# jc-bao/gym-formation

Hardware: AMD Instinct MI355X
Metric: env-steps/sec (higher is better)
Workload: dtype f32

## Files before the change

gym-formation_amd/csrc/fg_obs_writers.hpp:

```cpp
#ifndef FG_OBS_WRITERS_HPP_
#define FG_OBS_WRITERS_HPP_

#include "fg_common.hpp"

namespace fg {

template <class V2> FG_DEV V2 lds_if(bool c, const V2* __restrict__ p, int idx_if_true) {
    V2 t = p[c ? idx_if_true : 0];
    t.x = c ? t.x : 0.0f; t.y = c ? t.y : 0.0f;
    return t;
}

constexpr bool FG_ROWS_MERGED = true;
template <int NC, int NW, int E, int PACE = 0>
FG_DEV void write_obs_rows(const real2* __restrict__ tables0, int env_stride, int w,
                           real2* __restrict__ out_env0, size_t env_units, int El, int parts,
                           int wg_part = 0, int wg_parts = 1, bool pace_on = true) {
    constexpr int N = NC;
    constexpr int WPE = (E >= NW) ? 1 : NW / E;
    constexpr int ESTEP = (E >= NW) ? NW : 1;
    static_assert((E >= NW) ? (E % NW == 0) : (NW % E == 0), "waves and envs must tile");
    const int lane = threadIdx.x & 63;
    const int row0 = (E >= NW) ? 0 : w % WPE;
    constexpr unsigned ROWU = 3u * N;
    for (int ee = (E >= NW) ? w : w / WPE; ee < El; ee += (E >= NW ? ESTEP : E)) {
        const real2* __restrict__ AA = tables0 + (size_t)ee * env_stride;
        real2* __restrict__ out = out_env0 + (size_t)ee * env_units;
        if constexpr (N <= 64) {
            constexpr int RW = 64 / N;
            const int rsub = lane / N, u = lane - rsub * N;
            const bool act = rsub < RW;
            const real2 zero = make_real2(0.f, 0.f);
            const real2 Pm = lds_if(act && u >= 1, AA, u - 1);
            const real2 Pu = lds_if(act && u >= 1, AA, u);
            const int xoff = (u == 0) ? 4 * N : 0;
            constexpr int CS = (2 * N + 63) / 64;
            constexpr int RS = (2 * N <= 64) ? 64 / (2 * N) : 1;
            const int ssub = (2 * N <= 64) ? lane / (2 * N) : 0;
            const int sidx = (2 * N <= 64) ? lane - ssub * 2 * N : lane;
            real2 sv[CS];
#pragma unroll
            for (int c = 0; c < CS; ++c)
                sv[c] = lds_if(ssub < RS && sidx + 64 * c < 2 * N, AA, N + sidx + 64 * c);
#pragma unroll 2
            for (int rb = row0; rb < N; rb += RW * WPE) {
                const int r = rb + rsub * WPE;
                if ((parts & 1) && act && r < N) {
                    const real2 x = AA[xoff + r];
                    const real2 c = (u - 1 >= r) ? Pu : Pm;
                    out[(unsigned)r * ROWU + (unsigned)u] = make_real2(c.x - x.x, c.y - x.y);
                }
#pragma unroll
                for (int k0 = 0; k0 < RW; k0 += RS) {
                    const int rs = rb + (k0 + ssub) * WPE;
                    if ((parts & 2) && ssub < RS && k0 + ssub < RW && rs < N) {
#pragma unroll
                        for (int c = 0; c < CS; ++c)
                            if (sidx + 64 * c < 2 * N) out[(unsigned)rs * ROWU + (unsigned)(N + sidx + 64 * c)] = sv[c];
                    }
                }
            }
        } else if constexpr (FG_ROWS_MERGED && ((3 * N + 63) / 64 < (N + 63) / 64 + (2 * N + 63) / 64)) {
            constexpr int CR = (3 * N + 63) / 64;
            constexpr int C_MIX = N / 64;
            real2 Pm[CR], Pu[CR];
#pragma unroll
            for (int c = 0; c < CR; ++c) {
                const int u = lane + 64 * c;
                if (c <= C_MIX) {
                    const bool dyn = u >= 1 && u < N, stat = u >= N && u < 3 * N;
                    Pm[c] = lds_if(dyn || stat, AA, stat ? u : u - 1);
                    Pu[c] = lds_if(dyn || stat, AA, u);
                } else {
                    Pm[c] = Pu[c] = lds_if(u < 3 * N, AA, u);
                }
            }
            const int nshare = WPE * wg_parts, share = wg_part * WPE + row0;
            const int PER = (N + nshare - 1) / nshare;
            const int r_end = min(N, (share + 1) * PER);
#pragma unroll 2
            for (int r = share * PER; r < r_end; ++r) {
                const real2 xp = AA[r];
                const real2 x0 = AA[(lane == 0 ? 4 * N : 0) + r];
                real2* __restrict__ orow = out + (unsigned)r * ROWU;
#pragma unroll
                for (int c = 0; c < CR; ++c) {
                    const int u = lane + 64 * c;
                    real2 val;
                    if (c < C_MIX || (c == C_MIX && (N % 64) == 0)) {
                        const real2 x = (c == 0) ? x0 : xp;
                        const real2 cc = (u - 1 >= r) ? Pu[c] : Pm[c];
                        val = make_real2(cc.x - x.x, cc.y - x.y);
                    } else if (c == C_MIX) {
                        const bool dyn = u < N;
                        const real2 x = (c == 0) ? x0 : xp;
                        const real2 cc = (u - 1 >= r) ? Pu[c] : Pm[c];
                        val = make_real2(cc.x - (dyn ? x.x : 0.0f), cc.y - (dyn ? x.y : 0.0f));
                    } else {
                        val = Pu[c];
                    }
                    if (u < 3 * N) orow[u] = val;
                }
                if (PACE > 0 && pace_on) __builtin_amdgcn_s_sleep(PACE);
            }
        } else {
            constexpr int CD = (N + 63) / 64, CS = (2 * N + 63) / 64;
            const real2 zero = make_real2(0.f, 0.f);
            real2 Pm[CD], Pu[CD], sv[CS];
#pragma unroll
            for (int c = 0; c < CD; ++c) {
                const int u = lane + 64 * c;
                Pm[c] = lds_if(u >= 1 && u < N, AA, u - 1);
                Pu[c] = lds_if(u >= 1 && u < N, AA, u);
            }
#pragma unroll
            for (int c = 0; c < CS; ++c) sv[c] = lds_if(lane + 64 * c < 2 * N, AA, N + lane + 64 * c);
            const int nshare = WPE * wg_parts, share = wg_part * WPE + row0;
            const int PER = (N + nshare - 1) / nshare;
            const int r_end = min(N, (share + 1) * PER);
#pragma unroll 2
            for (int r = share * PER; r < r_end; ++r) {
                const real2 xp = AA[r];
                const real2 x0 = AA[(lane == 0 ? 4 * N : 0) + r];
                real2* __restrict__ orow = out + (unsigned)r * ROWU;
#pragma unroll
                for (int c = 0; c < CD; ++c) {
                    const int u = lane + 64 * c;
                    const real2 x = (c == 0) ? x0 : xp;
                    const real2 cc = (u - 1 >= r) ? Pu[c] : Pm[c];
                    if ((parts & 1) && u < N) orow[u] = make_real2(cc.x - x.x, cc.y - x.y);
                }
#pragma unroll
                for (int c = 0; c < CS; ++c)
                    if ((parts & 2) && lane + 64 * c < 2 * N) orow[N + lane + 64 * c] = sv[c];
                if (PACE > 0 && pace_on) __builtin_amdgcn_s_sleep(PACE);
            }
        }
    }
}

template <int NC, int RT> constexpr int tile_units() { return (3 * NC * RT + 16 + 2 + 1) & ~1; }

template <int NC, int NW, int E, int RT, bool STREAM>
FG_DEV void write_obs_tiled(const float2* __restrict__ tables0, int env_stride, int w, float2* __restrict__ tiles,
                            float2* __restrict__ out_env0, size_t unit0, size_t env_units, int El) {
    constexpr int N = NC;
    constexpr int WPE = (E >= NW) ? 1 : NW / E;
    static_assert((E >= NW) ? (E % NW == 0) : (NW % E == 0), "waves and envs must tile");
    static_assert(N <= 32 && N % RT == 0, "tiled writer: N <= 32, RT divides N");
    constexpr unsigned ROWU = 3u * N, TU = ROWU * RT;
    constexpr int TILES_ENV = N / RT;
    constexpr int MY_TILES = (TILES_ENV + WPE - 1) / WPE;
    const int lane = threadIdx.x & 63;
    float2* tile0 = tiles + w * 2 * tile_units<NC, RT>();
    constexpr int RW = 64 / N;
    const int rsub = lane / N, u = lane - rsub * N;
    const bool act = rsub < RW;
    const int xoff = (u == 0) ? 4 * N : 0;
    constexpr int RS = 64 / (2 * N);
    const int ssub = lane / (2 * N), sidx = lane - ssub * 2 * N;
    const int e_first = (E >= NW) ? w : w / WPE, e_step = (E >= NW) ? NW : E;
    const int t_first = (E >= NW) ? 0 : w % WPE;
    const int n_env = (El > e_first) ? (El - e_first + e_step - 1) / e_step : 0;
    const int total = n_env * MY_TILES;

    constexpr unsigned ENVU = ROWU * N;
    const unsigned pad = (unsigned)(env_units - ENVU);
    static_assert(!STREAM || (E >= NW && NC >= 16), "streaming form: waves own whole envs, rows of >= 16 units");
    const bool own = STREAM && ((unit0 & 15) == 0) && (pad == 0 || (pad < 16 && (env_units & 15) == 0));
    auto head_units = [&](int ee) -> unsigned {
        return (own && pad == 0) ? (16u - (unsigned)(((size_t)ee * env_units) & 15)) & 15u : 0u;
    };
    auto extra_units = [&](int ee) -> unsigned {
        if (!own) return 0u;
        if (pad) return pad;
        return (ee + 1 < El) ? head_units(ee + 1) : 0u;
    };

    int cur_env = -1;
    const float2* __restrict__ AA = tables0;
    float2 Pm = make_float2(0.f, 0.f), Pu = Pm, sv = Pm;
    auto locate = [&](int t, int& ee, int& r0) {
        const int ie = t / MY_TILES, it = t - ie * MY_TILES;
        ee = e_first + ie * e_step;
        r0 = (t_first + it * WPE) * RT;
    };
    auto compose = [&](int t) {
        int ee, r0; locate(t, ee, r0);
        if (r0 >= N) return;
        if (ee != cur_env) {
            cur_env = ee;
            AA = tables0 + (size_t)ee * env_stride;
            Pm = lds_if(act && u >= 1, AA, u - 1);
            Pu = lds_if(act && u >= 1, AA, u);
            sv = lds_if(ssub < RS, AA, N + sidx);
        }
        const unsigned par = (unsigned)((unit0 + (size_t)ee * env_units + (size_t)r0 * ROWU) & 1);
        float2* img = tile0 + (t & 1) * tile_units<NC, RT>() + par;
#pragma unroll
        for (int rb = 0; rb < RT; rb += RW) {
            const int rl = rb + rsub;
            if (act && rl < RT) {
                const int r = r0 + rl;
                const float2 x = AA[xoff + r];
                const float2 c = (u - 1 >= r) ? Pu : Pm;
                img[(unsigned)rl * ROWU + (unsigned)u] = make_float2(c.x - x.x, c.y - x.y);
            }
        }
#pragma unroll
        for (int rb = 0; rb < RT; rb += RS) {
            const int rl = rb + ssub;
            if (ssub < RS && rl < RT) img[(unsigned)rl * ROWU + (unsigned)(N + sidx)] = sv;
        }
        if (STREAM && r0 + RT == N) {
            const unsigned x = extra_units(ee);
            if ((unsigned)lane < x) {
                float2 val = make_float2(0.f, 0.f);
                if (pad == 0) {
                    static_assert(ROWU >= 16, "the line remainder must stay inside row 0 of the next env");
                    const float2* __restrict__ A1 = tables0 + (size_t)(ee + 1) * env_stride;
                    const float2 a = A1[lane == 0 ? 3 * N : lane], b = A1[0];
                    const bool rel = lane >= 1 && lane < N;
                    val = make_float2(a.x - (rel ? b.x : 0.f), a.y - (rel ? b.y : 0.f));
                }
                img[TU + (unsigned)lane] = val;
            }
        }
    };
    auto stream = [&](int t) {
        int ee, r0; locate(t, ee, r0);
        if (r0 >= N) return;
        const unsigned par = (unsigned)((unit0 + (size_t)ee * env_units + (size_t)r0 * ROWU) & 1);
        const float2* img = tile0 + (t & 1) * tile_units<NC, RT>() + par;
        float2* __restrict__ out = out_env0 + (size_t)ee * env_units + (size_t)r0 * ROWU;
        if constexpr (!STREAM) {
            if (par && lane == 0) out[0] = img[0];
            constexpr unsigned NPMAX = TU >> 1;
            const unsigned npair = (TU - par) >> 1;
            const f32x4* src4 = reinterpret_cast<const f32x4*>(img + par);
            f32x4* __restrict__ dst4 = reinterpret_cast<f32x4*>(out + par);
#pragma unroll
            for (unsigned q0 = 0; q0 < NPMAX; q0 += 64) {
                const unsigned q = q0 + lane;
                if (q < npair) dst4[q] = src4[q];
            }
            if (((TU - par) & 1u) && lane == 63) out[TU - 1] = img[TU - 1];
        } else {
            const unsigned s = (r0 == 0) ? head_units(ee) : 0u;
            const unsigned end = TU + ((r0 + RT == N) ? extra_units(ee) : 0u);
            const unsigned p2 = (par + s) & 1u;
            if (p2 && lane == 0) out[s] = img[s];
            constexpr unsigned NPMAX = (TU + 16) >> 1;
            const unsigned npair = (end - s - p2) >> 1;
            const f32x4* src4 = reinterpret_cast<const f32x4*>(img + s + p2);
            f32x4* __restrict__ dst4 = reinterpret_cast<f32x4*>(out + s + p2);
            constexpr unsigned NFULL = ((TU - 16) >> 1) / 64;
#pragma unroll
            for (unsigned c = 0; c < NFULL; ++c) {
                const f32x4 v = src4[c * 64 + lane];
                asm volatile("s_waitcnt lgkmcnt(0)" ::: "memory");
                dst4[c * 64 + lane] = v;
                asm volatile("" ::: "memory");
                __builtin_amdgcn_s_sleep(1);
            }
#pragma unroll
            for (unsigned q0 = NFULL * 64; q0 < NPMAX; q0 += 64) {
                const unsigned q = q0 + lane;
                if (q < npair) dst4[q] = src4[q];
            }
            if (((end - s - p2) & 1u) && lane == 63) out[end - 1] = img[end - 1];
        }
    };
    if (total > 0) compose(0);
    for (int t = 0; t < total; ++t) {
        if (t + 1 < total) compose(t + 1);
        stream(t);
    }
}

constexpr int FG_WR_GATHER = 64;
template <int NC> constexpr int gather_passes() { return (3 * NC * NC / 2 + 2 + 63) / 64; }
template <int NC> constexpr int gather_lut_units() { return 2 * gather_passes<NC>() * 64 * 2; }

template <int NC>
FG_DEV void build_gather_lut(uint4* __restrict__ lut, int t, int nthreads) {
    constexpr int N = NC, ROWU = 3 * N, TU = ROWU * N, P = gather_passes<NC>() * 64;
    static_assert(N >= 2 && 5 * N < 65536, "gather writer: table offsets are 16-bit, the table's zeros are the 0 operand");
    auto operands = [&](int unit, unsigned& a, unsigned& b) {
        const int r = unit / ROWU, u = unit - r * ROWU;
        if (u == 0) { a = N; b = 4 * N + r; }
        else if (u < N) { a = (u - 1 >= r) ? u : u - 1; b = r; }
        else { a = u; b = N; }
    };
    for (int e = t; e < 2 * P; e += nthreads) {
        const int par = e / P, q = e - par * P;
        const int npair = (TU - par) >> 1;
        const bool tail = ((TU - par) & 1) != 0;
        int unit = -1, kind = 0;
        if (q < npair) { unit = 2 * q + par; kind = 2; }
        else if (par && q == npair) { unit = 0; kind = 1; }
        else if (tail && q == npair + par) { unit = TU - 1; kind = 1; }
        unsigned a0 = N, b0 = N, a1 = N, b1 = N;
        if (kind >= 1) operands(unit, a0, b0);
        if (kind == 2) operands(unit + 1, a1, b1);
        lut[e] = make_uint4(a0 | (b0 << 16), a1 | (b1 << 16), (unsigned)(unit < 0 ? 0 : unit) | ((unsigned)kind << 16), 0u);
    }
}

template <int NC> struct GatherEntries {
    uint32_t ab0[gather_passes<NC>()], ab1[gather_passes<NC>()], dst[gather_passes<NC>()];
    int phase = -1;
};

template <int NC, int NW, int E>
FG_DEV void write_obs_gather(const float2* __restrict__ tables0, int env_stride, int w, const uint4* __restrict__ lut,
                             float2* __restrict__ out_env0, size_t unit0, size_t env_units, int El, GatherEntries<NC>& cache) {
    constexpr int PASSES = gather_passes<NC>(), P = PASSES * 64;
    const int lane = threadIdx.x & 63;
    for (int ee = w; ee < El; ee += NW) {
        const float2* __restrict__ T = tables0 + (size_t)ee * env_stride;
        const size_t first = unit0 + (size_t)ee * env_units;
        float2* __restrict__ out = out_env0 + (size_t)ee * env_units;
        const int phase = (int)(first & 1);
        if (phase != cache.phase) {
            const uint4* __restrict__ L = lut + phase * P + lane;
#pragma unroll
            for (int c = 0; c < PASSES; ++c) {
                const uint4 t = L[c * 64];
                cache.ab0[c] = t.x; cache.ab1[c] = t.y; cache.dst[c] = t.z;
            }
            cache.phase = phase;
        }
        f32x4 val[PASSES];
#pragma unroll
        for (int c = 0; c < PASSES; ++c) {
            const float2 A0 = T[cache.ab0[c] & 0xffffu], B0 = T[cache.ab0[c] >> 16], A1 = T[cache.ab1[c] & 0xffffu], B1 = T[cache.ab1[c] >> 16];
            val[c] = (f32x4){A0.x - B0.x, A0.y - B0.y, A1.x - B1.x, A1.y - B1.y};
        }
#pragma unroll
        for (int c = 0; c < PASSES; ++c) {
            const unsigned kind = cache.dst[c] >> 16, dst = cache.dst[c] & 0xffffu;
            if (kind == 2) *reinterpret_cast<f32x4*>(out + dst) = val[c];
            else if (kind == 1) out[dst] = make_float2(val[c].x, val[c].y);
        }
    }
}

template <int NC, int NW, int E, int CHMAX = 4> struct SpanGather {
    static constexpr int ENVU = 3 * NC * NC, PIECES = E * ENVU / 2, INSTR = (PIECES + 63) / 64, MINE = (INSTR + NW - 1) / NW;
    static_assert((E * ENVU) % 2 == 0, "an even number of units per workgroup span");
    static FG_DEV void setup(uint2* __restrict__ lut, int w, int env_stride) {
        const int lane = threadIdx.x & 63;
        auto operands = [&](int unit) -> uint32_t {
            const int e = unit / ENVU, q = unit - e * ENVU;
            const int r = q / (3 * NC), u = q - r * (3 * NC);
            uint32_t a, b;
            if (u == 0) { a = NC; b = 4 * NC + r; }
            else if (u < NC) { a = (u - 1 >= r) ? u : u - 1; b = r; }
            else { a = u; b = NC; }
            const uint32_t base = (uint32_t)(e * env_stride);
            return (a + base) | ((b + base) << 16);
        };
        for (int t = 0; t < MINE; ++t) {
            const int piece = (w + NW * t) * 64 + lane;
            if (piece < PIECES) lut[piece] = make_uint2(operands(2 * piece), operands(2 * piece + 1));
        }
    }
    static FG_DEV void write(const uint2* __restrict__ lut, const float2* __restrict__ tables0, int w, float2* __restrict__ out) {
        const int lane = threadIdx.x & 63;
        f32x4* const out4 = reinterpret_cast<f32x4*>(out);
        constexpr int CH = MINE < CHMAX ? MINE : CHMAX;
#pragma unroll
        for (int t0 = 0; t0 < MINE; t0 += CH) {
            uint2 ent[CH];
#pragma unroll
            for (int c = 0; c < CH; ++c) {
                const int piece = (w + NW * (t0 + c)) * 64 + lane;
                ent[c] = lut[(t0 + c < MINE && piece < PIECES) ? piece : 0];
            }
            f32x4 val[CH];
#pragma unroll
            for (int c = 0; c < CH; ++c) {
                const float2 A0 = tables0[ent[c].x & 0xffffu], B0 = tables0[ent[c].x >> 16];
                const float2 A1 = tables0[ent[c].y & 0xffffu], B1 = tables0[ent[c].y >> 16];
                val[c] = (f32x4){A0.x - B0.x, A0.y - B0.y, A1.x - B1.x, A1.y - B1.y};
            }
#pragma unroll
            for (int c = 0; c < CH; ++c) {
                const int piece = (w + NW * (t0 + c)) * 64 + lane;
                if (t0 + c < MINE && piece < PIECES) out4[piece] = val[c];
            }
        }
    }
};

}

#endif
```

gym-formation_amd/csrc/fg_rollout_kernels.hpp:

```cpp
#ifndef FG_ROLLOUT_KERNELS_HPP_
#define FG_ROLLOUT_KERNELS_HPP_

#include "fg_common.hpp"
#include "fg_pair_loops.hpp"
#include "fg_obs_writers.hpp"
#include "fg_policy_kernels.hpp"

namespace fg {

__host__ __device__ constexpr int roll_block_floats(int n) { return 20 * n + 6 * npad(n); }
template <int NC, int WR, int NWW, int E> constexpr int roll_writer_units() {
    if constexpr (WR == 0) return 0;
    else if constexpr (WR == FG_WR_GATHER)
        return gather_lut_units<NC>() > E * 3 * NC * NC / 2 ? gather_lut_units<NC>() : E * 3 * NC * NC / 2;
    else return 2 * NWW * tile_units<NC, WR - 1>();
}

template <int NC, int TW, int E, int WR, int PER> constexpr int roll_lds_base_bytes() {
    return E * roll_block_floats(NC) * (int)sizeof(real) + roll_writer_units<NC, WR, TW / 64, E>() * (int)sizeof(float2) +
           (PER > 0 ? E * policy_block_units(NC) * (int)sizeof(float2) : 0);
}
template <int NC, int E> constexpr int roll_rew_floats() { return 2 * 3 * E * NC; }
template <int NC, int TW, int E, int WR, int PER> constexpr bool roll_rew_in_lds() {
    return WR == FG_WR_GATHER &&
           roll_lds_base_bytes<NC, TW, E, WR, PER>() + roll_rew_floats<NC, E>() * (int)sizeof(float) <= 160 * 1024;
}
template <int NC, int TW, int E, int WR, int PER> constexpr int roll_lds_bytes() {
    return roll_lds_base_bytes<NC, TW, E, WR, PER>() +
           (roll_rew_in_lds<NC, TW, E, WR, PER>() ? roll_rew_floats<NC, E>() * (int)sizeof(float) : 0);
}

template <int NC, int G, int TP, int TW, int E, int WR, int PER = 0, bool STREAM = false>
__global__ __launch_bounds__(TP + TW) __attribute__((amdgpu_waves_per_eu((TP + TW) <= 512 && PER < 8 ? 4 : 3)))
void rollout_kernel(const Args a) {
    constexpr bool POLICY = PER > 0;
    static_assert(G <= 64 && E * G == TP && TW % 64 == 0 && TP % 64 == 0, "bad rollout geometry");
    constexpr int N = NC, NP = npad(NC), NWW = TW / 64;
    constexpr int NPS = NP <= 16 ? NP : 0;
    extern __shared__ __attribute__((aligned(16))) real2 smem[];
    real* const smemf = reinterpret_cast<real*>(smem);
    const int tid = threadIdx.x;
    const bool producer = tid < TP;
    const int e = producer ? tid / G : 0;
    const int i = tid % G;
    const int b0 = (int)blockIdx.x * E;
    const int b = b0 + e;
    const bool env_ok = producer && (b < a.B);
    const bool valid = env_ok && (i < N);
    const int El = min(E, a.B - b0);
    real* const blk = smemf + e * roll_block_floats(N);
    real2* const TB0 = reinterpret_cast<real2*>(blk);
    real* const QX = blk + 20 * N;
    real* const QY = QX + NP; real* const PX = QY + NP; real* const PY = PX + NP;
    real* const SX = PY + NP; real* const SY = SX + NP;

    const real one_minus_damp = 1.0f - a.p.damping;
    const real dt = a.p.dt;
    const real cutoff = a.p.dist_min + (FG_F64 ? 40.0f : 18.0f) * a.p.contact_margin;
    const real cutoff2 = cutoff * cutoff;
    const real thr2 = (real)((double)a.p.collide_thresh * (double)a.p.collide_thresh);
    const real invN = 1.0f / (real)N;
    const uint64_t rbase = rng_base(a.p);

    real2 p = make_real2(0.f, 0.f), v = p, s = p, iv = p;
    int t_step = 0;
    const size_t sidx = (size_t)b * N + i;
    if (valid) {
        p = make_real2(a.px[sidx], a.py[sidx]);
        v = make_real2(a.vx[sidx], a.vy[sidx]);
        s = reinterpret_cast<const real2*>(a.shape)[sidx];
        QX[i] = p.x; QY[i] = p.y; SX[i] = s.x; SY[i] = s.y;
        if (i < N - 1) { TB0[N + i] = make_real2(0.f, 0.f); TB0[5 * N + N + i] = make_real2(0.f, 0.f); }
    } else if (env_ok && i < NP) {
        QX[i] = FAR_AWAY; QY[i] = FAR_AWAY; PX[i] = FAR_AWAY; PY[i] = FAR_AWAY; SX[i] = FAR_AWAY; SY[i] = FAR_AWAY;
    }
    if (env_ok) { iv = reinterpret_cast<const real2*>(a.ivel)[b]; if (a.step) t_step = a.step[b]; }

    constexpr bool ACT4 = !POLICY && ((TP + TW) > 512 || WR == FG_WR_GATHER);
    real2 u_even = make_real2(0.f, 0.f), u_odd = u_even;
    const size_t act_stride = (size_t)a.B * N;
    const real2* const act0 = reinterpret_cast<const real2*>(a.act) + (valid ? sidx : 0);
    const real2* act_next = act0 + (a.K > 1 ? act_stride : 0);
    const uint32_t lane_off = valid ? (uint32_t)sidx : 0u;
    real2 cur[4], nxt[4];
#pragma unroll
    for (int t = 0; t < 4; ++t) { cur[t] = make_real2(0.f, 0.f); nxt[t] = cur[t]; }
    auto load_batch = [&](real2 (&dst)[4], int j0) {
        if (valid) {
#pragma unroll
            for (int t = 0; t < 4; ++t)
                dst[t] = (reinterpret_cast<const real2*>(a.act) + (size_t)min(j0 + t, a.K - 1) * act_stride)[lane_off];
        }
    };
    if constexpr (ACT4) load_batch(cur, 0);
    else if (!POLICY && valid) u_even = *act0;
    real2* const pol_tab = reinterpret_cast<real2*>(smemf + E * roll_block_floats(N)) + roll_writer_units<NC, WR, NWW, E>() +
                            e * policy_block_units(N);
    constexpr bool REWLDS = roll_rew_in_lds<NC, TW, E, WR, PER>();
    real* const rew_lds = smemf + roll_lds_base_bytes<NC, TW, E, WR, PER>() / (int)sizeof(real);

    auto produce = [&](int k, const real2& u_cur, real2& u_nxt) {
        real2* const A = TB0 + (k & 1) * 5 * N;
        __builtin_amdgcn_fence(__ATOMIC_ACQ_REL, "wavefront");
        real2 u_act = u_cur;
        if constexpr (POLICY) {
            if (valid) { pol_tab[i] = make_real2(p.x - QX[0], p.y - QY[0]); pol_tab[N + i] = s; }
            WaveSync()();
            const real2* res = bfs_policy_env<(PER > 0 ? PER : 3), policy_levels_ct<NC, (PER > 0 ? PER : 3)>()>(pol_tab, N, a.pl, iv, i, G, WaveSync());
            if (valid) {
                u_act = res[i];
                if (a.act_out) reinterpret_cast<real2*>(a.act_out)[((size_t)k * a.B + b) * N + i] = u_act;
            }
        }
        if (valid) {
            if constexpr (!POLICY && !ACT4) {
                u_nxt = *act_next;
                act_next += (k + 2 < a.K) ? act_stride : 0;
            }
            real2 f = contact_force_packed<NPS>(QX, QY, NP, i, p, a.p.contact_force, a.p.contact_margin,
                                                 a.p.dist_min, cutoff2);
            f.x += a.p.mass * (a.p.sensitivity * u_act.x);
            f.y += a.p.mass * (a.p.sensitivity * u_act.y);
            v.x = v.x * one_minus_damp + (f.x / a.p.mass) * dt;
            v.y = v.y * one_minus_damp + (f.y / a.p.mass) * dt;
            p.x += v.x * dt;
            p.y += v.y * dt;
            PX[i] = p.x; PY[i] = p.y;
        }
        t_step += 1;
        __builtin_amdgcn_fence(__ATOMIC_ACQ_REL, "wavefront");
        __builtin_amdgcn_wave_barrier();
        real sums[4] = {valid ? p.x : 0.f, valid ? p.y : 0.f, valid ? v.x : 0.f, valid ? v.y : 0.f};
        env_reduce<G, G, 4, R_SUM, R_SUM, R_SUM, R_SUM>(sums, nullptr);
        const real mx = sums[0] * invN, my = sums[1] * invN;
        const real mvx = sums[2] * invN, mvy = sums[3] * invN;
        real rowmin = INFINITY, colmin = INFINITY;
        int cnt = 0, arg_lm = 0, arg_ag = 0;
        if (valid)
            reward_pass_packed<false, NPS>(PX, PY, SX, SY, NP, p, p.x - mx, p.y - my, s.x + mx, s.y + my, thr2,
                                           rowmin, colmin, cnt, arg_lm, arg_ag);
        real red[3] = {valid ? rowmin : -INFINITY, valid ? colmin : -INFINITY, (real)cnt};
        env_reduce<G, G, 3, R_MAX, R_MAX, R_SUM, R_SUM>(red, nullptr);
        const real H = rsqrt_(rmax(red[0], red[1]));
        const real ex = iv.x - mvx, ey = iv.y - mvy;
        const real velterm = rsqrt_(ex * ex + ey * ey);
        const bool is_done = t_step >= a.p.world_length;
        if (valid) {
            const real shared = (real)(-(double)N * ((double)H + (double)velterm) - (double)red[2]);
            const real own = (-H - velterm) - (real)cnt;
            if constexpr (REWLDS) {
                real* const R = rew_lds + (k & 1) * 3 * E * N + e * N + i;
                R[0] = shared; R[E * N] = own; reinterpret_cast<uint32_t*>(R)[2 * E * N] = is_done ? 1u : 0u;
            } else {
                const size_t o = ((size_t)k * a.B + b) * N + i;
                if (a.rew) a.rew[o] = shared;
                if (a.indiv) a.indiv[o] = own;
                if (a.done) a.done[o] = is_done ? 1 : 0;
            }
        }
        if (a.p.auto_reset) {
            const bool mine = is_done && env_ok;
            if (__any(mine) != 0) {
                uint32_t c[4] = {(uint32_t)(b + a.p.env_index_base), (uint32_t)i, (uint32_t)(rbase + k),
                                 (uint32_t)((rbase + k) >> 32)};
                philox4x32(c, (uint32_t)a.p.seed, (uint32_t)(a.p.seed >> 32));
                real raw[2] = {valid ? u_pm1(c[2]) : 0.f, valid ? u_pm1(c[3]) : 0.f};
                const real rx = raw[0], ry = raw[1];
                env_reduce<G, G, 2, R_SUM, R_SUM, R_SUM, R_SUM>(raw, nullptr);
                uint32_t c2[4] = {(uint32_t)(b + a.p.env_index_base), 0xFFFFFFFFu, (uint32_t)(rbase + k),
                                  (uint32_t)((rbase + k) >> 32)};
                philox4x32(c2, (uint32_t)a.p.seed, (uint32_t)(a.p.seed >> 32));
                if (mine) {
                    iv = make_real2(u_pm1(c2[0]), u_pm1(c2[1]));
                    t_step = 0;
                    if (valid) {
                        p = make_real2(u_pm1(c[0]), u_pm1(c[1]));
                        v = make_real2(0.f, 0.f);
                        s = make_real2(rfma(-raw[0], invN, rx), rfma(-raw[1], invN, ry));
                        SX[i] = s.x; SY[i] = s.y;
                        int ir = i, br = b;
                        asm volatile("" : "+v"(ir), "+v"(br));
                        reinterpret_cast<real2*>(a.shape)[(size_t)br * N + ir] = s;
                        if (i == 0) reinterpret_cast<real2*>(a.ivel)[br] = iv;
                    }
                }
            }
        }
        if (valid) {
            A[i] = p; A[3 * N + i] = v; A[4 * N + i] = make_real2(-v.x, -v.y);
            A[2 * N - 1 + i] = s;
            if (i == 0) A[3 * N - 1] = iv;
            QX[i] = p.x; QY[i] = p.y;
        }
    };

    constexpr bool SPAN_OK = WR == FG_WR_GATHER && (E * 3 * NC * NC) % 2 == 0 && (E - 1) * (roll_block_floats(NC) / 2) + 5 * NC < 32768;
    using Span = SpanGather<(SPAN_OK ? NC : 2), NWW, (SPAN_OK ? E : 2), ((TP + TW) > 768 ? 1 : (TP + TW) <= 512 ? 2 : 4)>;
    uint2* const span_lut = reinterpret_cast<uint2*>(smemf + E * roll_block_floats(N));
    bool use_span = false;
    if constexpr (SPAN_OK)
        use_span = El == E && a.obs_pitch == 3LL * N * N && (((size_t)a.B * (size_t)a.obs_pitch) & 1) == 0 &&
                   (((size_t)b0 * (size_t)a.obs_pitch) & 1) == 0;
    if constexpr (WR == FG_WR_GATHER) {
        if (!producer) {
            if (use_span) Span::setup(span_lut, (tid - TP) >> 6, roll_block_floats(N) / 2);
            else build_gather_lut<NC>(reinterpret_cast<uint4*>(smemf + E * roll_block_floats(N)), tid - TP, TW);
        }
    }
    if (producer) __builtin_amdgcn_s_setprio(FG_PRODUCER_PRIO);
    if (producer) produce(0, ACT4 ? cur[0] : u_even, u_odd);
    __builtin_amdgcn_s_waitcnt(0x0F70);
    __syncthreads();
    auto pipeline_step = [&](int k, const real2& u_cur, real2& u_nxt) {
        if (producer) {
            if (k + 1 < a.K) produce(k + 1, u_cur, u_nxt);
        } else {
            if constexpr (REWLDS) {
                const real* const R = rew_lds + (k & 1) * 3 * E * N;
                const int cnt = El * N;
                const size_t o0 = ((size_t)k * a.B + b0) * N;
                int q0 = tid - TP;
                asm volatile("" : "+v"(q0));
                for (int q = q0; q < cnt; q += TW) {
                    if (a.rew) a.rew[o0 + q] = R[q];
                    if (a.indiv) a.indiv[o0 + q] = R[E * N + q];
                    if (a.done) a.done[o0 + q] = (uint8_t)reinterpret_cast<const uint32_t*>(R)[2 * E * N + q];
                }
            }
            int slot = k;
            bool want_obs = a.obs != nullptr;
            if (a.obs_every > 1) { want_obs = want_obs && ((k + 1) % a.obs_every == 0); slot = k / a.obs_every; }
            if (want_obs) {
                const size_t unit0 = ((size_t)slot * a.B + b0) * (size_t)a.obs_pitch;
                const size_t env_units = (size_t)a.obs_pitch;
                const real2* tables0 = reinterpret_cast<const real2*>(smemf) + (k & 1) * 5 * N;
                if constexpr (WR == 0)
                    write_obs_rows<NC, NWW, E>(tables0, roll_block_floats(N) / 2, (tid - TP) >> 6,
                                               reinterpret_cast<real2*>(a.obs) + unit0, env_units, El, 3);
                else if constexpr (WR == FG_WR_GATHER) {
                  if (use_span)
                    Span::write(span_lut, tables0, (tid - TP) >> 6, reinterpret_cast<real2*>(a.obs) + unit0);
                  else {
                    GatherEntries<(WR == FG_WR_GATHER ? NC : 2)> gather_entries;
                    write_obs_gather<NC, NWW, E>(tables0, roll_block_floats(N) / 2, (tid - TP) >> 6,
                                                 reinterpret_cast<const uint4*>(smemf + E * roll_block_floats(N)),
                                                 reinterpret_cast<real2*>(a.obs) + unit0, unit0, env_units, El, gather_entries);
                  }
                }
                else
                    write_obs_tiled<NC, NWW, E, WR - 1, STREAM>(tables0, roll_block_floats(N) / 2, (tid - TP) >> 6,
                                                                reinterpret_cast<real2*>(smemf + E * roll_block_floats(N)),
                                                                reinterpret_cast<real2*>(a.obs) + unit0, unit0, env_units, El);
            }
        }
        __syncthreads();
    };
    if constexpr (ACT4) {
        for (int k = 0; k < a.K; k += 4) {
            if (producer && k + 4 < a.K) load_batch(nxt, k + 4);
            pipeline_step(k, cur[1], u_odd);
            if (k + 1 < a.K) pipeline_step(k + 1, cur[2], u_odd);
            if (k + 2 < a.K) pipeline_step(k + 2, cur[3], u_odd);
            if (k + 3 < a.K) pipeline_step(k + 3, nxt[0], u_odd);
#pragma unroll
            for (int t = 0; t < 4; ++t) cur[t] = nxt[t];
        }
    } else {
        for (int k = 0; k < a.K; k += 2) {
            pipeline_step(k, u_odd, u_even);
            if (k + 1 < a.K) pipeline_step(k + 1, u_even, u_odd);
        }
    }
    if (valid) {
        int is = i, bs = b;
        asm volatile("" : "+v"(is), "+v"(bs));
        const size_t so = (size_t)bs * N + is;
        a.px[so] = p.x; a.py[so] = p.y; a.vx[so] = v.x; a.vy[so] = v.y;
    }
    if (a.step && env_ok && i == 0) a.step[b] = t_step;
}

template <int NC, int A, int E, int TW, int PER = 0, bool BATCHES = false>
__global__ __launch_bounds__(E * 64 + TW) void rollout_kernel_wide(const Args a) {
    constexpr bool POLICY = PER > 0;
    static_assert(!(BATCHES && POLICY), "the batch-pipelined single step takes its actions from the caller");
    static_assert(A * 64 >= NC && (A - 1) * 64 < NC && TW % 64 == 0, "bad wide rollout geometry");
    constexpr int N = NC, NP = npad(NC), NWW = TW / 64, TP = E * 64;
    extern __shared__ __attribute__((aligned(16))) real2 smem[];
    real* const smemf = reinterpret_cast<real*>(smem);
    const int tid = threadIdx.x, lane = tid & 63;
    const int wave = __builtin_amdgcn_readfirstlane(tid >> 6);
    const bool producer = wave < E;
    const int e = producer ? wave : 0;
    const int NG = BATCHES ? max(1, a.groups) : 1;
    const int wg0 = blockIdx.x * E * NG;
    int b = wg0 + e;
    bool env_ok = producer && (b < a.B);
    real* const blk = smemf + e * roll_block_floats(N);
    real2* const TB0 = reinterpret_cast<real2*>(blk);
    real* const QX = blk + 20 * N;
    real* const QY = QX + NP; real* const PX = QY + NP; real* const PY = PX + NP;
    real* const SX = PY + NP; real* const SY = SX + NP;

    const real one_minus_damp = 1.0f - a.p.damping;
    const real dt = a.p.dt;
    const real cutoff = a.p.dist_min + (FG_F64 ? 40.0f : 18.0f) * a.p.contact_margin;
    const real cutoff2 = cutoff * cutoff;
    const real thr2 = (real)((double)a.p.collide_thresh * (double)a.p.collide_thresh);
    const real invN = 1.0f / (real)N;
    const real inv_k = 1.0f / a.p.contact_margin;
    const uint64_t rbase = rng_base(a.p);

    real2 p[A], v[A], s[A];
    real2 u_pre[A];
    auto valid = [&](int q) { return env_ok && (q < A - 1 || lane < N - 64 * (A - 1)); };
    real2 iv = make_real2(0.f, 0.f);
    int t_step = 0;
    if (producer) {
#pragma unroll
        for (int q = 0; q < A; ++q) {
            const int i = lane + 64 * q;
            if (i < N - 1) { TB0[N + i] = make_real2(0.f, 0.f); TB0[5 * N + N + i] = make_real2(0.f, 0.f); }
            if (i >= N && i < NP) {
                QX[i] = FAR_AWAY; QY[i] = FAR_AWAY; PX[i] = FAR_AWAY; PY[i] = FAR_AWAY; SX[i] = FAR_AWAY; SY[i] = FAR_AWAY;
            }
        }
    }
    auto load_group = [&](int g) {
        b = wg0 + g * E + e;
        env_ok = producer && (b < a.B);
#pragma unroll
        for (int q = 0; q < A; ++q) {
            const int i = lane + 64 * q;
            p[q] = v[q] = s[q] = make_real2(0.f, 0.f);
            if (valid(q)) {
                const size_t o = (size_t)b * N + i;
                p[q] = make_real2(a.px[o], a.py[o]);
                v[q] = make_real2(a.vx[o], a.vy[o]);
                s[q] = reinterpret_cast<const real2*>(a.shape)[o];
                QX[i] = p[q].x; QY[i] = p[q].y; SX[i] = s[q].x; SY[i] = s[q].y;
            }
        }
        iv = make_real2(0.f, 0.f); t_step = 0;
        if (env_ok) { iv = reinterpret_cast<const real2*>(a.ivel)[b]; if (a.step) t_step = a.step[b]; }
    };
    auto load_actions = [&](int k) {
#pragma unroll
        for (int q = 0; q < A; ++q) {
            u_pre[q] = make_real2(0.f, 0.f);
            if (valid(q)) u_pre[q] = reinterpret_cast<const real2*>(a.act)[((size_t)k * a.B + b) * N + lane + 64 * q];
        }
    };
    auto store_group = [&]() {
#pragma unroll
        for (int q = 0; q < A; ++q) {
            if (valid(q)) {
                const size_t o = (size_t)b * N + lane + 64 * q;
                a.px[o] = p[q].x; a.py[o] = p[q].y; a.vx[o] = v[q].x; a.vy[o] = v[q].y;
            }
        }
        if (a.step && env_ok && lane == 0) a.step[b] = t_step;
    };

    real2* const pol_tab = reinterpret_cast<real2*>(smemf + E * roll_block_floats(N)) + e * policy_block_units(N);
    auto produce = [&](int k, int buf) {
        real2* const T = TB0 + buf * 5 * N;
        __builtin_amdgcn_fence(__ATOMIC_ACQ_REL, "wavefront");
        const real2* pol_res = nullptr;
        if constexpr (POLICY) {
#pragma unroll
            for (int q = 0; q < A; ++q) {
                const int i = lane + 64 * q;
                if (valid(q)) { pol_tab[i] = make_real2(p[q].x - QX[0], p[q].y - QY[0]); pol_tab[N + i] = s[q]; }
            }
            WaveSync()();
            pol_res = bfs_policy_env<(PER > 0 ? PER : 3), policy_levels_ct<NC, (PER > 0 ? PER : 3)>()>(pol_tab, N, a.pl, iv, lane, 64, WaveSync());
        }
        real2 u_cur[A];
        if constexpr (!POLICY) {
#pragma unroll
            for (int q = 0; q < A; ++q) u_cur[q] = u_pre[q];
            if constexpr (!BATCHES) load_actions(min(k + 1, a.K - 1));
        }
        real fx[A], fy[A];
#pragma unroll
        for (int q = 0; q < A; ++q) { fx[q] = 0.f; fy[q] = 0.f; }
        if (env_ok) {
            for (int j = 0; j < NP; j += 2) {
                const realx2 qx = *reinterpret_cast<const realx2*>(QX + j);
                const realx2 qy = *reinterpret_cast<const realx2*>(QY + j);
#pragma unroll
                for (int q = 0; q < A; ++q) {
                    const int i = lane + 64 * q;
                    const realx2 dx = (realx2){p[q].x, p[q].x} - qx, dy = (realx2){p[q].y, p[q].y} - qy;
                    const realx2 d2 = dx * dx + dy * dy;
                    const bool n0 = (d2.x < cutoff2) && (j != i) && valid(q);
                    const bool n1 = (d2.y < cutoff2) && (j + 1 != i) && valid(q);
                    if (n0 || n1) {
                        auto add = [&](real ddx, real ddy, real dd2) {
                            const real d = hw_sqrt(dd2);
                            const real x = (a.p.dist_min - d) * inv_k;
                            const real pen = a.p.contact_margin * (rmax(x, real(0)) + hw_log(1.0f + hw_exp(-rabs(x))));
                            const real c = a.p.contact_force * pen * hw_rcp(d);
                            fx[q] += ddx * c; fy[q] += ddy * c;
                        };
                        if (n0) add(dx.x, dy.x, d2.x);
                        if (n1) add(dx.y, dy.y, d2.y);
                    }
                }
            }
        }
        real sums[4] = {0.f, 0.f, 0.f, 0.f};
        real part[A][4];
#pragma unroll
        for (int q = 0; q < A; ++q) {
            part[q][0] = part[q][1] = part[q][2] = part[q][3] = 0.f;
            if (valid(q)) {
                const int i = lane + 64 * q;
                real2 u;
                if constexpr (POLICY) {
                    u = pol_res[i];
                    if (a.act_out) reinterpret_cast<real2*>(a.act_out)[((size_t)k * a.B + b) * N + i] = u;
                } else {
                    u = u_cur[q];
                }
                const real ffx = fx[q] + a.p.mass * (a.p.sensitivity * u.x);
                const real ffy = fy[q] + a.p.mass * (a.p.sensitivity * u.y);
                v[q].x = v[q].x * one_minus_damp + (ffx / a.p.mass) * dt;
                v[q].y = v[q].y * one_minus_damp + (ffy / a.p.mass) * dt;
                p[q].x += v[q].x * dt;
                p[q].y += v[q].y * dt;
                PX[i] = p[q].x; PY[i] = p[q].y;
                part[q][0] = p[q].x; part[q][1] = p[q].y; part[q][2] = v[q].x; part[q][3] = v[q].y;
            }
        }
        t_step += 1;
        __builtin_amdgcn_fence(__ATOMIC_ACQ_REL, "wavefront");
        __builtin_amdgcn_wave_barrier();
#pragma unroll
        for (int q = 0; q < A; ++q) {
            env_reduce<64, 64, 4, R_SUM, R_SUM, R_SUM, R_SUM>(part[q], nullptr);
            if (q == 0) { sums[0] = part[0][0]; sums[1] = part[0][1]; sums[2] = part[0][2]; sums[3] = part[0][3]; }
            else { sums[0] += part[q][0]; sums[1] += part[q][1]; sums[2] += part[q][2]; sums[3] += part[q][3]; }
        }
        const real mx = sums[0] * invN, my = sums[1] * invN;
        const real mvx = sums[2] * invN, mvy = sums[3] * invN;
        real rowmin[A], colmin[A];
        int cnt[A];
#pragma unroll
        for (int q = 0; q < A; ++q) { rowmin[q] = INFINITY; colmin[q] = INFINITY; cnt[q] = -1; }
        if (env_ok) {
            for (int j = 0; j < NP; j += 2) {
                const realx2 qx = *reinterpret_cast<const realx2*>(PX + j);
                const realx2 qy = *reinterpret_cast<const realx2*>(PY + j);
                const realx2 sx = *reinterpret_cast<const realx2*>(SX + j);
                const realx2 sy = *reinterpret_cast<const realx2*>(SY + j);
#pragma unroll
                for (int q = 0; q < A; ++q) {
                    const realx2 cx = qx - (realx2){p[q].x, p[q].x}, cy = qy - (realx2){p[q].y, p[q].y};
                    const realx2 dc = cx * cx + cy * cy;
                    cnt[q] += (dc.x < thr2 ? 1 : 0) + (dc.y < thr2 ? 1 : 0);
                    const real ptx = p[q].x - mx, pty = p[q].y - my;
                    const realx2 rx = (realx2){ptx, ptx} - sx, ry = (realx2){pty, pty} - sy;
                    const realx2 dr = rx * rx + ry * ry;
                    const real tx = s[q].x + mx, ty = s[q].y + my;
                    const realx2 ux = qx - (realx2){tx, tx}, uy = qy - (realx2){ty, ty};
                    const realx2 dq = ux * ux + uy * uy;
                    rowmin[q] = rmin(rmin(rowmin[q], dr.x), dr.y);
                    colmin[q] = rmin(rmin(colmin[q], dq.x), dq.y);
                }
            }
        }
        real red[3] = {-INFINITY, -INFINITY, 0.f};
#pragma unroll
        for (int q = 0; q < A; ++q) {
            if (valid(q)) {
                cnt[q] += (thr2 > 0.0f ? 0 : 1);
                red[0] = rmax(red[0], rowmin[q]); red[1] = rmax(red[1], colmin[q]); red[2] += (real)cnt[q];
            }
        }
        env_reduce<64, 64, 3, R_MAX, R_MAX, R_SUM, R_SUM>(red, nullptr);
        const real H = rsqrt_(rmax(red[0], red[1]));
        const real ex = iv.x - mvx, ey = iv.y - mvy;
        const real velterm = rsqrt_(ex * ex + ey * ey);
        const bool is_done = t_step >= a.p.world_length;
        const real shared = (real)(-(double)N * ((double)H + (double)velterm) - (double)red[2]);
#pragma unroll
        for (int q = 0; q < A; ++q) {
            if (valid(q)) {
                const size_t o = ((size_t)k * a.B + b) * N + lane + 64 * q;
                if (a.rew) a.rew[o] = shared;
                if (a.indiv) a.indiv[o] = (-H - velterm) - (real)cnt[q];
                if (a.done) a.done[o] = is_done ? 1 : 0;
            }
        }
        if (a.p.auto_reset && is_done && env_ok) {
            real raw[2] = {0.f, 0.f};
            real rawp[A][2];
            real rx[A], ry[A];
            uint32_t c0[A], c1[A];
#pragma unroll
            for (int q = 0; q < A; ++q) {
                uint32_t c[4] = {(uint32_t)(b + a.p.env_index_base), (uint32_t)(lane + 64 * q), (uint32_t)(rbase + k),
                                 (uint32_t)((rbase + k) >> 32)};
                philox4x32(c, (uint32_t)a.p.seed, (uint32_t)(a.p.seed >> 32));
                c0[q] = c[0]; c1[q] = c[1];
                rx[q] = valid(q) ? u_pm1(c[2]) : 0.f; ry[q] = valid(q) ? u_pm1(c[3]) : 0.f;
                rawp[q][0] = rx[q]; rawp[q][1] = ry[q];
            }
#pragma unroll
            for (int q = 0; q < A; ++q) {
                env_reduce<64, 64, 2, R_SUM, R_SUM, R_SUM, R_SUM>(rawp[q], nullptr);
                if (q == 0) { raw[0] = rawp[0][0]; raw[1] = rawp[0][1]; } else { raw[0] += rawp[q][0]; raw[1] += rawp[q][1]; }
            }
            uint32_t c2[4] = {(uint32_t)(b + a.p.env_index_base), 0xFFFFFFFFu, (uint32_t)(rbase + k),
                              (uint32_t)((rbase + k) >> 32)};
            philox4x32(c2, (uint32_t)a.p.seed, (uint32_t)(a.p.seed >> 32));
            iv = make_real2(u_pm1(c2[0]), u_pm1(c2[1]));
            t_step = 0;
#pragma unroll
            for (int q = 0; q < A; ++q) {
                if (valid(q)) {
                    const int i = lane + 64 * q;
                    const size_t o = (size_t)b * N + i;
                    p[q] = make_real2(u_pm1(c0[q]), u_pm1(c1[q]));
                    v[q] = make_real2(0.f, 0.f);
                    s[q] = make_real2(rfma(-raw[0], invN, rx[q]), rfma(-raw[1], invN, ry[q]));
                    SX[i] = s[q].x; SY[i] = s[q].y;
                    reinterpret_cast<real2*>(a.shape)[o] = s[q];
                }
            }
            if (lane == 0) reinterpret_cast<real2*>(a.ivel)[b] = iv;
        }
#pragma unroll
        for (int q = 0; q < A; ++q) {
            if (valid(q)) {
                const int i = lane + 64 * q;
                T[i] = p[q]; T[3 * N + i] = v[q]; T[4 * N + i] = make_real2(-v[q].x, -v[q].y);
                T[2 * N - 1 + i] = s[q];
                QX[i] = p[q].x; QY[i] = p[q].y;
            }
        }
        if (env_ok && lane == 0) T[3 * N - 1] = iv;
    };

    constexpr bool per_step = BATCHES;
    const int total = per_step ? NG : a.K;
    if (producer) {
        load_group(0);
        if constexpr (!POLICY) load_actions(0);
        produce(0, 0); if (per_step) store_group();
        __syncthreads();
        for (int it = 0; it < total; ++it) {
            if (it + 1 < total) {
                if (per_step) { load_group(it + 1); load_actions(0); produce(0, (it + 1) & 1); store_group(); }
                else produce(it + 1, (it + 1) & 1);
            }
            __syncthreads();
        }
        if (!per_step) store_group();
    } else {
        const int w = wave - E;
        __syncthreads();
        for (int it = 0; it < total; ++it) {
            const int k = per_step ? 0 : it;
            const int b0 = wg0 + (per_step ? it * E : 0);
            const int El = min(E, a.B - b0);
            int slot = k;
            bool want_obs = a.obs != nullptr && El > 0;
            if (a.obs_every > 1) { want_obs = want_obs && ((k + 1) % a.obs_every == 0); slot = k / a.obs_every; }
            if (want_obs) {
                const size_t unit0 = ((size_t)slot * a.B + b0) * (size_t)a.obs_pitch;
                write_obs_rows<NC, NWW, E>(reinterpret_cast<const real2*>(smemf) + (it & 1) * 5 * N,
                                           roll_block_floats(N) / 2, w,
                                           reinterpret_cast<real2*>(a.obs) + unit0, (size_t)a.obs_pitch, El, 3);
            }
            __syncthreads();
        }
    }
}

}

#endif
```

Measured before the change: 351.7 million.

## Carry the last observation tile's store across rollout steps in the tiled writer

Adds a cross-step pipelined form of the streaming tiled observation writer. The store of the previous step's final tile is deferred into the next step, where it overlaps with composing the first tile, and a drain call after the step loop writes the last one. This is meant to hide the store tail of each step's observation write behind the next step's work. It applies only to the N=27, E=16 streaming configuration. It adds bookkeeping for tile-buffer parity and alignment ownership across slots, which could corrupt output if the shared-memory tiles or offsets disagree.

Result: slower. 347.9 million (-1.1%).

```diff
diff --git a/gym-formation_amd/csrc/fg_obs_writers.hpp b/gym-formation_amd/csrc/fg_obs_writers.hpp
--- a/gym-formation_amd/csrc/fg_obs_writers.hpp
+++ b/gym-formation_amd/csrc/fg_obs_writers.hpp
@@ -141,9 +141,10 @@
 
 template <int NC, int RT> constexpr int tile_units() { return (3 * NC * RT + 16 + 2 + 1) & ~1; }
 
-template <int NC, int NW, int E, int RT, bool STREAM>
+template <int NC, int NW, int E, int RT, bool STREAM, bool CARRY = false>
 FG_DEV void write_obs_tiled(const float2* __restrict__ tables0, int env_stride, int w, float2* __restrict__ tiles,
-                            float2* __restrict__ out_env0, size_t unit0, size_t env_units, int El) {
+                            float2* __restrict__ out_env0, size_t unit0, size_t env_units, int El,
+                            int slot = 0, size_t back = 0, bool drain = false) {
     constexpr int N = NC;
     constexpr int WPE = (E >= NW) ? 1 : NW / E;
     static_assert((E >= NW) ? (E % NW == 0) : (NW % E == 0), "waves and envs must tile");
@@ -167,7 +168,7 @@
     constexpr unsigned ENVU = ROWU * N;
     const unsigned pad = (unsigned)(env_units - ENVU);
     static_assert(!STREAM || (E >= NW && NC >= 16), "streaming form: waves own whole envs, rows of >= 16 units");
-    const bool own = STREAM && ((unit0 & 15) == 0) && (pad == 0 || (pad < 16 && (env_units & 15) == 0));
+    bool own = STREAM && ((unit0 & 15) == 0) && (pad == 0 || (pad < 16 && (env_units & 15) == 0));
     auto head_units = [&](int ee) -> unsigned {
         return (own && pad == 0) ? (16u - (unsigned)(((size_t)ee * env_units) & 15)) & 15u : 0u;
     };
@@ -185,7 +186,7 @@
         ee = e_first + ie * e_step;
         r0 = (t_first + it * WPE) * RT;
     };
-    auto compose = [&](int t) {
+    auto compose = [&](int t, int g) {
         int ee, r0; locate(t, ee, r0);
         if (r0 >= N) return;
         if (ee != cur_env) {
@@ -196,7 +197,7 @@
             sv = lds_if(ssub < RS, AA, N + sidx);
         }
         const unsigned par = (unsigned)((unit0 + (size_t)ee * env_units + (size_t)r0 * ROWU) & 1);
-        float2* img = tile0 + (t & 1) * tile_units<NC, RT>() + par;
+        float2* img = tile0 + (g & 1) * tile_units<NC, RT>() + par;
 #pragma unroll
         for (int rb = 0; rb < RT; rb += RW) {
             const int rl = rb + rsub;
@@ -227,12 +228,12 @@
             }
         }
     };
-    auto stream = [&](int t) {
+    auto stream = [&](int t, int g, size_t bk) {
         int ee, r0; locate(t, ee, r0);
         if (r0 >= N) return;
-        const unsigned par = (unsigned)((unit0 + (size_t)ee * env_units + (size_t)r0 * ROWU) & 1);
-        const float2* img = tile0 + (t & 1) * tile_units<NC, RT>() + par;
-        float2* __restrict__ out = out_env0 + (size_t)ee * env_units + (size_t)r0 * ROWU;
+        const unsigned par = (unsigned)((unit0 - bk + (size_t)ee * env_units + (size_t)r0 * ROWU) & 1);
+        const float2* img = tile0 + (g & 1) * tile_units<NC, RT>() + par;
+        float2* __restrict__ out = out_env0 - bk + (size_t)ee * env_units + (size_t)r0 * ROWU;
         if constexpr (!STREAM) {
             if (par && lane == 0) out[0] = img[0];
             constexpr unsigned NPMAX = TU >> 1;
@@ -271,10 +272,26 @@
             if (((end - s - p2) & 1u) && lane == 63) out[end - 1] = img[end - 1];
         }
     };
-    if (total > 0) compose(0);
-    for (int t = 0; t < total; ++t) {
-        if (t + 1 < total) compose(t + 1);
-        stream(t);
+    if constexpr (!CARRY) {
+        if (total > 0) compose(0, 0);
+        for (int t = 0; t < total; ++t) {
+            if (t + 1 < total) compose(t + 1, t + 1);
+            stream(t, t, 0);
+        }
+    } else {
+        static_assert(STREAM, "the cross-step pipeline is a form of the streaming writer");
+        if (total <= 0) return;
+        const int g0 = slot * total;
+        if (drain) { stream(total - 1, g0 + total - 1, 0); return; }
+        const bool own_here = own;
+        const bool own_prev = (((unit0 - back) & 15) == 0) && (pad == 0 || (pad < 16 && (env_units & 15) == 0));
+        for (int t = -1; t + 1 < total; ++t) {
+            compose(t + 1, g0 + t + 1);
+            const bool pend = t < 0;
+            if (pend) own = own_prev;
+            if (!pend || slot > 0) stream(pend ? total - 1 : t, g0 + t, pend ? back : (size_t)0);
+            own = own_here;
+        }
     }
 }
 
diff --git a/gym-formation_amd/csrc/fg_rollout_kernels.hpp b/gym-formation_amd/csrc/fg_rollout_kernels.hpp
--- a/gym-formation_amd/csrc/fg_rollout_kernels.hpp
+++ b/gym-formation_amd/csrc/fg_rollout_kernels.hpp
@@ -211,6 +211,7 @@
     if (producer) produce(0, ACT4 ? cur[0] : u_even, u_odd);
     __builtin_amdgcn_s_waitcnt(0x0F70);
     __syncthreads();
+    constexpr bool XSTEP = STREAM && NC == 27 && WR != 0 && WR != FG_WR_GATHER && !POLICY && E == 16;
     auto pipeline_step = [&](int k, const real2& u_cur, real2& u_nxt) {
         if (producer) {
             if (k + 1 < a.K) produce(k + 1, u_cur, u_nxt);
@@ -248,9 +249,10 @@
                   }
                 }
                 else
-                    write_obs_tiled<NC, NWW, E, WR - 1, STREAM>(tables0, roll_block_floats(N) / 2, (tid - TP) >> 6,
-                                                                reinterpret_cast<real2*>(smemf + E * roll_block_floats(N)),
-                                                                reinterpret_cast<real2*>(a.obs) + unit0, unit0, env_units, El);
+                    write_obs_tiled<NC, NWW, E, WR - 1, STREAM, XSTEP>(tables0, roll_block_floats(N) / 2, (tid - TP) >> 6,
+                                                                       reinterpret_cast<real2*>(smemf + E * roll_block_floats(N)),
+                                                                       reinterpret_cast<real2*>(a.obs) + unit0, unit0, env_units, El,
+                                                                       slot, (size_t)a.B * (size_t)a.obs_pitch);
             }
         }
         __syncthreads();
@@ -269,6 +271,16 @@
         for (int k = 0; k < a.K; k += 2) {
             pipeline_step(k, u_odd, u_even);
             if (k + 1 < a.K) pipeline_step(k + 1, u_even, u_odd);
+        }
+    }
+    if constexpr (XSTEP) {
+        const int nslot = a.obs_every > 1 ? a.K / a.obs_every : a.K;
+        if (!producer && a.obs != nullptr && nslot > 0) {
+            const size_t unit0 = ((size_t)(nslot - 1) * a.B + b0) * (size_t)a.obs_pitch;
+            write_obs_tiled<NC, NWW, E, WR - 1, STREAM, true>(reinterpret_cast<const real2*>(smemf), roll_block_floats(N) / 2, (tid - TP) >> 6,
+                                                              reinterpret_cast<real2*>(smemf + E * roll_block_floats(N)),
+                                                              reinterpret_cast<real2*>(a.obs) + unit0, unit0, (size_t)a.obs_pitch, El,
+                                                              nslot - 1, 0, true);
         }
     }
     if (valid) {
diff --git a/profiles/r06_cross_step_ab.py b/profiles/r06_cross_step_ab.py
--- /dev/null
+++ b/profiles/r06_cross_step_ab.py
@@ -0,0 +1,79 @@
+#!/usr/bin/env python3
+import hashlib
+import os
+import sys
+
+ROOT = os.path.dirname(os.path.dirname(os.path.abspath(__file__)))
+sys.path[:0] = [ROOT, os.path.join(ROOT, "gym-formation_amd")]
+import torch
+import formation_gym
+from formation_gym import _native
+
+split = sys.argv.index("--")
+arms = [a.split("=", 1) for a in sys.argv[1:split]]
+shapes = [tuple(int(x) for x in s.split(":")) for s in sys.argv[split + 1:]]
+ROUNDS = int(os.environ.get("FG_AB_ROUNDS", "3"))
+dev = "cuda:0"
+
+
+def use(path):
+    _native.LIB_PATH = os.path.abspath(path)
+    _native._lib = None
+    return _native.load()
+
+
+def make_env(N, B):
+    env = formation_gym.make_env("formation_hd_env", False, N, num_envs=B, device=dev)
+    env.scenario.seed(3)
+    env.scenario.reset_device(env.world, rng_offset=1)
+    env.auto_reset = True
+    env.world.step_count.copy_((torch.arange(B, dtype=torch.int32, device=dev) * 7) % 100)
+    return env
+
+
+for N, B, K in shapes:
+    gen = torch.Generator(device=dev); gen.manual_seed(5)
+    acts = torch.rand((K, B, N, 2), device=dev, generator=gen) * 2 - 1
+    use(arms[0][1])
+    owner = make_env(N, B)
+    out = owner.alloc_rollout_buffers(K, candidates=int(os.environ.get("FG_AB_CANDIDATES", "8")),
+                                      max_arena_bytes=int(float(os.environ.get("FG_AB_ARENA_GB", "192")) * (1 << 30)))
+    pl = owner.placement or {}
+    envs = {}
+    for name, path in arms:
+        use(path)
+        envs[name] = make_env(N, B)
+        envs[name].rollout(acts, out=out)
+        torch.cuda.synchronize()
+        h = hashlib.sha256()
+        for k in ("obs", "reward", "indiv", "done"):
+            h.update(out[k].cpu().numpy().tobytes())
+        h.update(envs[name].world.pos_x.cpu().numpy().tobytes())
+        print("%d x %d x %d arm %-8s digest %s  placed %s" % (N, B, K, name, h.hexdigest()[:16],
+                                                             [pl.get("arena_GB"), pl.get("kept")]), flush=True)
+    reps = max(3, int(20e3 / (K * max(1.0, 24e-6 * N * N * B / 6.0))))
+    med = {name: [] for name, _ in arms}
+    for rnd in range(ROUNDS):
+        for name, _ in arms:
+            env = envs[name]
+            for _ in range(3):
+                env.rollout(acts, out=out)
+            torch.cuda.synchronize()
+            blocks = []
+            for _ in range(7):
+                e0, e1 = torch.cuda.Event(enable_timing=True), torch.cuda.Event(enable_timing=True)
+                e0.record()
+                for _ in range(reps):
+                    env.rollout(acts, out=out)
+                e1.record()
+                torch.cuda.synchronize()
+                blocks.append(e0.elapsed_time(e1) / reps / K * 1e3)
+            blocks.sort()
+            med[name].append(blocks[3])
+            print("%d x %d x %d round %d arm %-8s %.3f us/step (min %.3f max %.3f)" % (N, B, K, rnd + 1, name, blocks[3], blocks[0], blocks[-1]),
+                  flush=True)
+    print("%d x %d x %d summary: %s" % (N, B, K, "  ".join(
+        "%s %.3f (%.3f-%.3f)" % (n, sorted(v)[len(v) // 2], min(v), max(v)) for n, v in med.items())), flush=True)
+    use(arms[0][1])
+    del envs, out, acts, owner
+    torch.cuda.empty_cache()
```
